# elfi-dev/elfi

Hardware: AMD Instinct MI355X
Metric: ABC distances/sec (higher is better)
Workload: dtype f64; 1 GPU; configs[1]: synthetic Gaussian summaries, 1000000 samples x 32 summaries per GPU per step, elfi.Distance('euclidean'), inputs resident in HBM; samples_per_gpu=1000000, summaries=32, layout=row-major (n,m) f64, batches_in_rotation=3, exchange=none (N = 1), exchange_every=8, world_size_seen=1

## Files before the change

### elfi_amd/csrc/adaptive.hip

```cpp
#include "common.hpp"
#include "tile_stream.hpp"
#include "internal.hpp"
#include "dist_launch.hpp"

#include <algorithm>

#pragma clang fp contract(off)

namespace elfihip {

constexpr int ADA_T = 256;
constexpr int ADA_U = 8;
constexpr int ADA_RMAX = 128;
constexpr int ADA_OCC = 4;

struct AdaptArgs {
  RowArgs A;
  const double* acc;
  unsigned long long* acc_count;
  double* partial;
};

struct ColStat {
  double n, mean, M2;
};

__device__ __forceinline__ void chan_merge(ColStat& a, double nb, double mb, double qb) {
  if (nb == 0.0) return;
  if (a.n == 0.0) {
    a.n = nb;
    a.mean = mb;
    a.M2 = qb;
    return;
  }
  const double tot = a.n + nb;
  const double delta = mb - a.mean;
  const double f = nb / tot;
  a.M2 = a.M2 + qb + delta * delta * (a.n * f);
  a.mean = a.mean + delta * f;
  a.n = tot;
}

typedef const double __attribute__((address_space(4))) * cdptr;
__device__ __forceinline__ cdptr as_constant(const double* p) { return (cdptr) reinterpret_cast<uintptr_t>(p); }

template <int B, bool PRE>
__device__ __forceinline__ double row_distance(const double* row, cdptr ys, cdptr w, int m) {
  double s = 0.0;
  double wn[B], yn[PRE ? 1 : B];
#pragma unroll
  for (int i = 0; i < B; ++i) {
    wn[i] = w[i];
    if constexpr (!PRE) yn[i] = ys[i];
  }
  double xn[4];
#pragma unroll
  for (int i = 0; i < 4; ++i) xn[i] = row[i];
  int j0 = 0;
  for (; j0 + B <= m; j0 += B) {
    double wc[B], yc[PRE ? 1 : B];
#pragma unroll
    for (int i = 0; i < B; ++i) {
      wc[i] = wn[i];
      if constexpr (!PRE) yc[i] = yn[i];
    }
    const int jn = j0 + 2 * B <= m ? j0 + B : j0;
#pragma unroll
    for (int i = 0; i < B; ++i) {
      wn[i] = w[jn + i];
      if constexpr (!PRE) yn[i] = ys[jn + i];
    }
#pragma unroll
    for (int i0 = 0; i0 < B; i0 += 4) {
      double x[4];
#pragma unroll
      for (int i = 0; i < 4; ++i) x[i] = xn[i];
#pragma unroll
      for (int i = 0; i < 4; ++i) xn[i] = row[j0 + i0 + 4 + i];
#pragma unroll
      for (int i = 0; i < 4; ++i) {
        double d = x[i];
        if constexpr (!PRE) d = d - yc[i0 + i];
        const double d2 = d * d;
        s = s + wc[i0 + i] * d2;
      }
    }
  }
  for (int j = j0; j < m; ++j) {
    double d = row[j];
    if constexpr (!PRE) d = d - ys[j];
    const double d2 = d * d;
    s = s + w[j] * d2;
  }
  return sqrt(s);
}

template <int CH>
__device__ __forceinline__ void chunk_stats(const double (&x)[CH], double& mean, double& q) {
  if constexpr (CH >= 4) {
    double a[4] = {0.0, 0.0, 0.0, 0.0};
#pragma unroll
    for (int i = 0; i < CH; i += 4) {
      a[0] += x[i];
      a[1] += x[i + 1];
      a[2] += x[i + 2];
      a[3] += x[i + 3];
    }
    mean = ((a[0] + a[1]) + (a[2] + a[3])) * (1.0 / CH);
    double b[4] = {0.0, 0.0, 0.0, 0.0};
#pragma unroll
    for (int i = 0; i < CH; i += 4) {
#pragma unroll
      for (int u = 0; u < 4; ++u) {
        const double e = x[i + u] - mean;
        b[u] += e * e;
      }
    }
    q = (b[0] + b[1]) + (b[2] + b[3]);
  } else {
    double a = 0.0;
#pragma unroll
    for (int i = 0; i < CH; ++i) a += x[i];
    mean = a * (1.0 / CH);
    q = 0.0;
#pragma unroll
    for (int i = 0; i < CH; ++i) {
      const double e = x[i] - mean;
      q += e * e;
    }
  }
}

template <int NU>
__global__ __launch_bounds__(ADA_T, ADA_OCC) void adaptive_pass_kernel(AdaptArgs P) {
  extern __shared__ __align__(16) double lds[];
  constexpr int U = NU > 0 ? NU : ADA_U;
  constexpr bool POW2 = NU > 0;
  const RowArgs& A = P.A;
  const int T = ADA_T, tid = threadIdx.x, m = A.m, K = A.K, R = A.R, mp = A.mp;
  double* tile = lds;
  const int tile_doubles = R * mp > 6 * T ? R * mp : 6 * T;
  double* accs = tile + tile_doubles + 8;
  int* flag = reinterpret_cast<int*>(accs + K);
  const cdptr ys = as_constant(A.y), ws = as_constant(A.aux);
  if (P.acc)
    for (int j = tid; j < K; j += T) accs[j] = P.acc[j];
  const int64_t ntiles = (A.n + R - 1) / R;
  const double inf = __longlong_as_double(0x7ff0000000000000ll);
  const double thr = A.F.thr ? *A.F.thr : inf;
  const int wave = __builtin_amdgcn_readfirstlane(tid >> 6);
  const int RB = R > 64 ? 2 : 1;
  const int CG = 4 / RB;
  const int rb = wave % RB, cg = wave / RB;
  const int rl = rb * 64 + (tid & 63);
  const bool owner = cg == (K - 1) % CG;
  unsigned long long nacc = 0;
  const int h = m >> 1;
  const int q0 = POW2 ? tid / h : 0, jj0 = POW2 ? tid - q0 * h : 0, QS = POW2 ? T / h : 1;
  const int64_t soff = (int64_t)q0 * A.ldx + 2 * jj0, sstep = (int64_t)QS * A.ldx;
  const int doff = q0 * mp + 2 * jj0, dstep = QS * mp;
  double2 yp = make_double2(0.0, 0.0);
  if constexpr (POW2) yp = make_double2(A.y[2 * jj0], A.y[2 * jj0 + 1]);
  const int G = T / m;
  const int g = tid / m, c = tid - g * m;
  const bool stats = P.partial != nullptr;
  ColStat st0 = {0.0, 0.0, 0.0}, st1 = {0.0, 0.0, 0.0};
  double2 v[U];
  auto fetch = [&](int64_t row0, int rows) {
    if constexpr (POW2) {
      const double* __restrict__ src = A.X + row0 * A.ldx + soff;
      if (rows == R) {
        if (A.nt) {
          typedef double v2d_nt __attribute__((ext_vector_type(2)));
#pragma unroll
          for (int u = 0; u < U; ++u) {
            const v2d_nt tv = __builtin_nontemporal_load(reinterpret_cast<const v2d_nt*>(src + u * sstep));
            v[u] = make_double2(tv.x, tv.y);
          }
        } else {
#pragma unroll
          for (int u = 0; u < U; ++u) v[u] = *reinterpret_cast<const double2*>(src + u * sstep);
        }
      } else {
#pragma unroll
        for (int u = 0; u < U; ++u) {
          v[u] = make_double2(0.0, 0.0);
          if (q0 + u * QS < rows) v[u] = *reinterpret_cast<const double2*>(src + u * sstep);
        }
      }
    } else {
      tile_fetch<U>(A, row0, rows, v);
    }
  };
  auto commit = [&](int rows) {
    if constexpr (POW2) {
      if (rows == R) {
#pragma unroll
        for (int u = 0; u < U; ++u) {
          double* dst = tile + doff + u * dstep;
          dst[0] = v[u].x - yp.x;
          dst[1] = v[u].y - yp.y;
        }
        if (stats) {
          double a[U], b[U], ma, qa, mb, qb;
#pragma unroll
          for (int u = 0; u < U; ++u) {
            a[u] = v[u].x;
            b[u] = v[u].y;
          }
          chunk_stats<U>(a, ma, qa);
          chunk_stats<U>(b, mb, qb);
          chan_merge(st0, (double)U, ma, qa);
          chan_merge(st1, (double)U, mb, qb);
        }
      } else {
        int cnt = 0;
        double sa = 0.0, sb = 0.0;
#pragma unroll
        for (int u = 0; u < U; ++u)
          if (q0 + u * QS < rows) {
            double* dst = tile + doff + u * dstep;
            dst[0] = v[u].x - yp.x;
            dst[1] = v[u].y - yp.y;
            sa += v[u].x;
            sb += v[u].y;
            ++cnt;
          }
        if (stats && cnt > 0) {
          const double ma = sa / (double)cnt, mb = sb / (double)cnt;
          double qa = 0.0, qb = 0.0;
#pragma unroll
          for (int u = 0; u < U; ++u)
            if (q0 + u * QS < rows) {
              const double ea = v[u].x - ma, eb = v[u].y - mb;
              qa += ea * ea;
              qb += eb * eb;
            }
          chan_merge(st0, (double)cnt, ma, qa);
          chan_merge(st1, (double)cnt, mb, qb);
        }
      }
    } else {
      tile_commit<U>(A, tile, rows, v);
    }
  };
  int64_t t = blockIdx.x;
  if (t < ntiles) fetch(t * R, (int)((A.n - t * R) < R ? (A.n - t * R) : R));
  for (; t < ntiles; t += gridDim.x) {
    const int64_t row0 = t * R;
    const int rows = (int)((A.n - row0) < R ? (A.n - row0) : R);
    __syncthreads();
    commit(rows);
    const int64_t tn = t + gridDim.x;
    if (tn < ntiles) fetch(tn * R, (int)((A.n - tn * R) < R ? (A.n - tn * R) : R));
    __syncthreads();
    double dlast = 0.0;
    bool ok = rl < rows;
    if (rl < rows) {
      const double* row = tile + (size_t)rl * mp;
      for (int k = cg; k < K; k += CG) {
        double r;
        if constexpr (POW2)
          r = row_distance<16, true>(row, ys, ws + (size_t)k * m, m);
        else
          r = row_distance<8, false>(row, ys, ws + (size_t)k * m, m);
        if (A.out) A.out[(row0 + rl) * K + k] = r;
        if (P.acc) ok = ok && r <= accs[k];
        dlast = r;
      }
    }
    if (P.acc && K > 1) {
      if (!owner) flag[cg * ADA_RMAX + rl] = ok ? 1 : 0;
      __syncthreads();
      if (owner) {
        const int ng = K < CG ? K : CG;
        for (int q = 0; q < ng; ++q)
          if (q != cg) ok = ok && flag[q * ADA_RMAX + rl] != 0;
      }
    }
    if (owner) {
      if (P.acc) nacc += (unsigned long long)__popcll(__ballot(ok));
      if (A.F.thr) reject_offer(A.F, ok && dlast < thr, dlast, A.F.row_base + row0 + rl);
    }
    if constexpr (!POW2) {
      if (stats && g < G && g < rows) {
        const double* col = tile + c;
        double sum = 0.0;
        int cnt = 0;
#pragma unroll 8
        for (int r = g; r < rows; r += G) {
          sum += col[(size_t)r * mp];
          ++cnt;
        }
        const double mt = sum / (double)cnt;
        double q = 0.0;
#pragma unroll 8
        for (int r = g; r < rows; r += G) {
          const double e = col[(size_t)r * mp] - mt;
          q += e * e;
        }
        chan_merge(st0, (double)cnt, mt, q);
      }
    }
  }
  if (stats) {
    __syncthreads();
    double* red = tile;
    const int nslot = POW2 ? QS : G;
    if constexpr (POW2) {
      double* e0 = red + 3 * ((size_t)q0 * m + 2 * jj0);
      e0[0] = st0.n, e0[1] = st0.mean, e0[2] = st0.M2;
      e0[3] = st1.n, e0[4] = st1.mean, e0[5] = st1.M2;
    } else if (g < G) {
      double* e0 = red + 3 * ((size_t)g * m + c);
      e0[0] = st0.n, e0[1] = st0.mean, e0[2] = st0.M2;
    }
    __syncthreads();
    if (tid < m) {
      ColStat a = {0.0, 0.0, 0.0};
      for (int sl = 0; sl < nslot; ++sl) {
        const double* e = red + 3 * ((size_t)sl * m + tid);
        chan_merge(a, e[0], e[1], e[2]);
      }
      double* o = P.partial + (size_t)blockIdx.x * (1 + 2 * m);
      if (tid == 0) o[0] = a.n;
      o[1 + tid] = a.mean;
      o[1 + m + tid] = a.M2;
    }
  }
  if (P.acc && (tid & 63) == 0 && nacc) atomicAdd(P.acc_count, nacc);
}

constexpr int ADA_NARROW_KMAX = 8;
constexpr int ADA_NARROW_U = 8;

template <int M, int U>
__global__ __launch_bounds__(256) void adaptive_narrow_kernel(AdaptArgs P) {
  __shared__ double rn[256], rm[256 * M], rq[256 * M];
  __shared__ __align__(16) double stage_all[4 * 64 * ADA_NARROW_KMAX];
  const RowArgs& A = P.A;
  const int tid = threadIdx.x, K = A.K;
  double* stage = stage_all + (tid >> 6) * 64 * ADA_NARROW_KMAX;
  const bool staged = A.out && (reinterpret_cast<uintptr_t>(A.out) & 15u) == 0;
  double yv[M], wv[ADA_NARROW_KMAX][M], accs[ADA_NARROW_KMAX];
#pragma unroll
  for (int j = 0; j < M; ++j) yv[j] = A.y[j];
#pragma unroll
  for (int k = 0; k < ADA_NARROW_KMAX; ++k) {
    accs[k] = (P.acc && k < K) ? P.acc[k] : 0.0;
#pragma unroll
    for (int j = 0; j < M; ++j) wv[k][j] = k < K ? A.aux[k * M + j] : 0.0;
  }
  const double inf = __longlong_as_double(0x7ff0000000000000ll);
  const double thr = A.F.thr ? *A.F.thr : inf;
  const bool stats = P.partial != nullptr;
  ColStat st[M];
#pragma unroll
  for (int j = 0; j < M; ++j) st[j] = {0.0, 0.0, 0.0};
  unsigned long long nacc = 0;
  typedef double v2d_nt __attribute__((ext_vector_type(2)));
  const int64_t per = 256 * U;
  for (int64_t base = (int64_t)blockIdx.x * per; base < A.n; base += (int64_t)gridDim.x * per) {
    double x[U][M];
#pragma unroll
    for (int u = 0; u < U; ++u) {
      const int64_t r = base + u * 256 + tid;
      const v2d_nt* src = reinterpret_cast<const v2d_nt*>(A.X + (r < A.n ? r : A.n - 1) * A.ldx);
#pragma unroll
      for (int h = 0; h < M / 2; ++h) {
        const v2d_nt t = __builtin_nontemporal_load(src + h);
        x[u][2 * h] = t.x;
        x[u][2 * h + 1] = t.y;
      }
    }
    if (stats) {
      if (base + per <= A.n) {
#pragma unroll
        for (int j = 0; j < M; ++j) {
          double col[U], mean, q;
#pragma unroll
          for (int u = 0; u < U; ++u) col[u] = x[u][j];
          chunk_stats<U>(col, mean, q);
          chan_merge(st[j], (double)U, mean, q);
        }
      } else {
        int cnt = 0;
#pragma unroll
        for (int u = 0; u < U; ++u) cnt += (base + u * 256 + tid < A.n) ? 1 : 0;
        if (cnt > 0) {
#pragma unroll
          for (int j = 0; j < M; ++j) {
            double sum = 0.0;
#pragma unroll
            for (int u = 0; u < U; ++u)
              if (base + u * 256 + tid < A.n) sum += x[u][j];
            const double mean = sum / (double)cnt;
            double q = 0.0;
#pragma unroll
            for (int u = 0; u < U; ++u)
              if (base + u * 256 + tid < A.n) {
                const double e = x[u][j] - mean;
                q += e * e;
              }
            chan_merge(st[j], (double)cnt, mean, q);
          }
        }
      }
    }
#pragma unroll
    for (int u = 0; u < U; ++u) {
      const int64_t r = base + u * 256 + tid;
      const bool live = r < A.n;
      double d2[M];
#pragma unroll
      for (int j = 0; j < M; ++j) {
        const double d = x[u][j] - yv[j];
        d2[j] = d * d;
      }
      double dlast = 0.0, dk[ADA_NARROW_KMAX];
      bool ok = live;
#pragma unroll
      for (int k = 0; k < ADA_NARROW_KMAX; ++k) {
        dk[k] = 0.0;
        if (k < K) {
          double sk = 0.0;
#pragma unroll
          for (int j = 0; j < M; ++j) sk = sk + wv[k][j] * d2[j];
          dlast = sqrt(sk);
          dk[k] = dlast;
          if (A.out && !staged && live) A.out[r * K + k] = dlast;
          if (P.acc) ok = ok && dlast <= accs[k];
        }
      }
      if (staged) {
        const int64_t r0 = base + u * 256 + (tid & ~63);
        const int64_t left = A.n - r0;
        if (left > 0) wave_store_rows<ADA_NARROW_KMAX>(stage, A.out + r0 * K, dk, K, tid & 63, left < 64 ? (int)left : 64);
      }
      if (P.acc) nacc += (unsigned long long)__popcll(__ballot(ok));
      if (A.F.thr) reject_offer(A.F, ok && dlast < thr, dlast, A.F.row_base + r);
    }
  }
  if (stats) {
    rn[tid] = st[0].n;
#pragma unroll
    for (int j = 0; j < M; ++j) {
      rm[j * 256 + tid] = st[j].mean;
      rq[j * 256 + tid] = st[j].M2;
    }
    __syncthreads();
    for (int s = 128; s > 0; s >>= 1) {
      double nb = 0.0;
      if (tid < s) nb = rn[tid + s];
      if (tid < s) {
#pragma unroll
        for (int j = 0; j < M; ++j) {
          ColStat a = {rn[tid], rm[j * 256 + tid], rq[j * 256 + tid]};
          chan_merge(a, nb, rm[j * 256 + tid + s], rq[j * 256 + tid + s]);
          rm[j * 256 + tid] = a.mean;
          rq[j * 256 + tid] = a.M2;
          if (j == M - 1) st[0].n = a.n;
        }
      }
      __syncthreads();
      if (tid < s) rn[tid] = st[0].n;
      __syncthreads();
    }
    if (tid < M) {
      double* o = P.partial + (size_t)blockIdx.x * (1 + 2 * M);
      if (tid == 0) o[0] = rn[0];
      o[1 + tid] = rm[tid * 256];
      o[1 + M + tid] = rq[tid * 256];
    }
  }
  if (P.acc && (tid & 63) == 0 && nacc) atomicAdd(P.acc_count, nacc);
}

__global__ __launch_bounds__(256) void adaptive_finish_kernel(const double* partial, int nparts, int m, double* bst,
                                                              double* state, unsigned* done) {
  __shared__ double rn[256], rm[256], rq[256];
  const int c = blockIdx.x, j = threadIdx.x, ns = 1 + 2 * m;
  ColStat a = {0.0, 0.0, 0.0};
  for (int p = j; p < nparts; p += 256) {
    const double* e = partial + (size_t)p * ns;
    chan_merge(a, e[0], e[1 + c], e[1 + m + c]);
  }
  rn[j] = a.n;
  rm[j] = a.mean;
  rq[j] = a.M2;
  __syncthreads();
  for (int s = 128; s > 0; s >>= 1) {
    if (j < s) {
      chan_merge(a, rn[j + s], rm[j + s], rq[j + s]);
      rn[j] = a.n;
      rm[j] = a.mean;
      rq[j] = a.M2;
    }
    __syncthreads();
  }
  if (j == 0) {
    if (c == 0) bst[0] = a.n;
    bst[1 + c] = a.mean;
    bst[1 + m + c] = a.M2;
    if (state) {
      const double n_old = state[0];
      ColStat f = {n_old, state[1 + c], state[1 + m + c]};
      if (n_old == 0.0) f.mean = 0.0, f.M2 = 0.0;
      chan_merge(f, a.n, a.mean, a.M2);
      state[1 + c] = f.mean;
      state[1 + m + c] = f.M2;
      const unsigned old = __hip_atomic_fetch_add(done, 1u, __ATOMIC_RELAXED, __HIP_MEMORY_SCOPE_AGENT);
      if (old + 1u == (unsigned)m) {
        state[0] = f.n;
        __hip_atomic_store(done, 0u, __ATOMIC_RELAXED, __HIP_MEMORY_SCOPE_AGENT);
      }
    }
  }
}

static size_t ada_lds_bytes(int m, int K, int R) {
  const int mp = m | 1;
  const size_t tile = std::max<size_t>((size_t)R * mp, 6 * (size_t)ADA_T);
  return (tile + 8 + (size_t)K + 2 * ADA_RMAX) * sizeof(double);
}

static int ada_rows_per_tile(int m) {
  int R = 2 * ADA_T * ADA_U / m;
  return R > ADA_RMAX ? ADA_RMAX : R;
}

static bool adaptive_narrow(const double* dX, int m, int64_t ldx, int K) {
  return (m == 2 || m == 4) && K >= 1 && K <= ADA_NARROW_KMAX && !(ldx & 1) && aligned16(dX);
}

bool adaptive_pass_supported(const double* dX, int m, int64_t ldx, int K) {
  if (adaptive_narrow(dX, m, ldx, K)) return true;
  if (m < 4 || m > ADA_T / 2 || (m & 1) || (ldx & 1) || !aligned16(dX)) return false;
  return ada_lds_bytes(m, K, ada_rows_per_tile(m)) <= 64 * 1024;
}

int adaptive_max_parts(const elfihip_ctx* ctx) { return ctx->cu_count * 8; }

int adaptive_pass_impl(elfihip_ctx* ctx, const double* dX, int64_t n, int m, int64_t ldx, const double* dy,
                       const double* dW, int K, double* dout, const RejectFilter* F, const double* dacc,
                       unsigned long long* dacc_count, double* partial, int* nparts) {
  if (nparts) *nparts = 0;
  if (n <= 0) return ELFIHIP_OK;
  AdaptArgs P;
  RowArgs& A = P.A;
  A = make_row_args(ctx, dX, n, m, ldx, dy, dW, 2.0, dout);
  A.K = K;
  A.R = ada_rows_per_tile(m);
  if (F) A.F = *F;
  P.acc = dacc;
  P.acc_count = dacc_count;
  P.partial = partial;
  if (adaptive_narrow(dX, m, ldx, K)) {
    constexpr int U = ADA_NARROW_U;
    int64_t gn = (n + 256 * U - 1) / (256 * U);
    if (gn > (int64_t)ctx->cu_count * 4) gn = (int64_t)ctx->cu_count * 4;
    if (m == 2)
      hipLaunchKernelGGL((adaptive_narrow_kernel<2, U>), dim3((unsigned)gn), dim3(256), 0, ctx->stream, P);
    else
      hipLaunchKernelGGL((adaptive_narrow_kernel<4, U>), dim3((unsigned)gn), dim3(256), 0, ctx->stream, P);
    if (nparts && partial) *nparts = (int)gn;
    return launch_status(ctx, "adaptive_narrow_kernel");
  }
  const size_t lds = ada_lds_bytes(m, K, A.R);
  const int64_t ntiles = (n + A.R - 1) / A.R;
  int per_cu = (int)((160 * 1024) / lds);
  if (per_cu > 8) per_cu = 8;
  if (per_cu < 1) per_cu = 1;
  int64_t g = (int64_t)ctx->cu_count * per_cu;
  if (g > ntiles) g = ntiles;
  if (g < 1) g = 1;
  const int h = m / 2;
  const int nu = (ADA_T % h == 0 && A.R % (ADA_T / h) == 0) ? A.R / (ADA_T / h) : 0;
#define ELFIHIP_ADA_LAUNCH(NU) \
  hipLaunchKernelGGL((adaptive_pass_kernel<NU>), dim3((unsigned)g), dim3(ADA_T), lds, ctx->stream, P)
  switch (nu) {
    case 8: ELFIHIP_ADA_LAUNCH(8); break;
    case 4: ELFIHIP_ADA_LAUNCH(4); break;
    case 2: ELFIHIP_ADA_LAUNCH(2); break;
    case 1: ELFIHIP_ADA_LAUNCH(1); break;
    default: ELFIHIP_ADA_LAUNCH(0); break;
  }
#undef ELFIHIP_ADA_LAUNCH
  if (nparts && partial) *nparts = (int)g;
  return launch_status(ctx, "adaptive_pass_kernel");
}

int adaptive_stats_finish(elfihip_ctx* ctx, const double* partial, int nparts, int m, double* bst, double* dstate) {
  if (nparts <= 0) return ELFIHIP_OK;
  if (dstate && !ctx->fold_cnt) {
    ELFIHIP_CHECK_HIP(ctx, hipMalloc(reinterpret_cast<void**>(&ctx->fold_cnt), 64));
    ELFIHIP_CHECK_HIP(ctx, hipMemsetAsync(ctx->fold_cnt, 0, 64, ctx->stream));
  }
  hipLaunchKernelGGL(adaptive_finish_kernel, dim3((unsigned)m), dim3(256), 0, ctx->stream, partial, nparts, m, bst, dstate,
                     ctx->fold_cnt);
  return launch_status(ctx, "adaptive statistics kernel");
}

}

using namespace elfihip;

extern "C" {

int elfihip_adaptive_push_dev(elfihip_ctx* ctx, elfihip_reject* state, const double* dX, int64_t n, int m, int64_t ldx,
                              const double* dy, const double* dW, int K, double* dout, double* dwelford,
                              int64_t row_base) {
  if (!ctx) return fail(nullptr, ELFIHIP_ERR_ARG, "ctx is NULL");
  ELFIHIP_REQUIRE(ctx, n >= 0 && m >= 1 && ldx >= m, "bad shape n=%lld m=%d ldx=%lld", (long long)n, m, (long long)ldx);
  ELFIHIP_REQUIRE(ctx, K >= 1 && K <= 64, "K=%d outside [1,64]", K);
  ELFIHIP_REQUIRE(ctx, n == 0 || (dX && dy && dW), "NULL data pointer");
  ELFIHIP_REQUIRE(ctx, !state || reject_ctx(state) == ctx, "the sampler state belongs to another context");
  if (n == 0) return ELFIHIP_OK;
  DeviceGuard g(ctx->device);
  return adaptive_push_impl(ctx, state, dX, n, m, ldx, dy, dW, K, dout, dwelford, row_base);
}

static int adaptive_push_host(elfihip_ctx* ctx, elfihip_reject* state, const double* X, int64_t n, int m, int64_t ldx,
                              const double* y, const double* W, int K, double* out, int64_t* count, double* mean,
                              double* M2, int64_t row_base) {
  ELFIHIP_REQUIRE(ctx, K >= 1 && K <= 64, "K=%d outside [1,64]", K);
  ELFIHIP_REQUIRE(ctx, y && W, "NULL data pointer");
  ELFIHIP_REQUIRE(ctx, (!count && !mean && !M2) || (count && mean && M2), "count / mean / M2 come together");
  ELFIHIP_REQUIRE(ctx, !state || reject_ctx(state) == ctx, "the sampler state belongs to another context");
  if (n == 0) return out ? keep_distances(ctx, nullptr, 0, K) : ELFIHIP_OK;
  DeviceGuard g(ctx->device);
  hipStream_t st = ctx->stream;
  const size_t ns = 1 + 2 * (size_t)m;
  std::vector<double> hst(ns, 0.0);
  if (count) {
    hst[0] = (double)*count;
    memcpy(&hst[1], mean, (size_t)m * sizeof(double));
    memcpy(&hst[1 + m], M2, (size_t)m * sizeof(double));
  }
  ELFIHIP_CHECK_HIP(ctx, ctx->par.reserve(((size_t)m + (size_t)K * m + ns) * sizeof(double)));
  double* dy = ctx->par.as<double>();
  double* dW = dy + m;
  double* dstate = dW + (size_t)K * m;
  ELFIHIP_CHECK_HIP(ctx, hipMemcpyAsync(dy, y, (size_t)m * sizeof(double), hipMemcpyHostToDevice, st));
  ELFIHIP_CHECK_HIP(ctx, hipMemcpyAsync(dW, W, (size_t)K * m * sizeof(double), hipMemcpyHostToDevice, st));
  if (count) ELFIHIP_CHECK_HIP(ctx, hipMemcpyAsync(dstate, hst.data(), ns * sizeof(double), hipMemcpyHostToDevice, st));
  double* dX;
  int64_t ldd;
  if (X) {
    ldd = (m + 1) & ~1;
    ELFIHIP_CHECK_HIP(ctx, ctx->in.reserve((size_t)n * ldd * sizeof(double)));
    dX = ctx->in.as<double>();
    ELFIHIP_CHECK_HIP(ctx, hipMemcpy2DAsync(dX, (size_t)ldd * sizeof(double), X, (size_t)ldx * sizeof(double),
                                            (size_t)m * sizeof(double), (size_t)n, hipMemcpyHostToDevice, st));
  } else {
    dX = ctx->rows.as<double>();
    ldd = m;
  }
  double* dout = nullptr;
  if (out) {
    ELFIHIP_CHECK_HIP(ctx, ctx->out.reserve((size_t)n * K * sizeof(double)));
    dout = ctx->out.as<double>();
  }
  ELFIHIP_TRY(adaptive_push_impl(ctx, state, dX, n, m, ldd, dy, dW, K, dout, count ? dstate : nullptr, row_base));
  if (out) {
    ELFIHIP_TRY(keep_distances(ctx, dout, n, K));
    ELFIHIP_CHECK_HIP(ctx, hipMemcpyAsync(out, dout, (size_t)n * K * sizeof(double), hipMemcpyDeviceToHost, st));
  }
  if (count) ELFIHIP_CHECK_HIP(ctx, hipMemcpyAsync(hst.data(), dstate, ns * sizeof(double), hipMemcpyDeviceToHost, st));
  ELFIHIP_CHECK_HIP(ctx, hipStreamSynchronize(st));
  if (count) {
    *count = (int64_t)hst[0];
    memcpy(mean, &hst[1], (size_t)m * sizeof(double));
    memcpy(M2, &hst[1 + m], (size_t)m * sizeof(double));
  }
  return ELFIHIP_OK;
}

int elfihip_adaptive_push(elfihip_ctx* ctx, elfihip_reject* state, const double* X, int64_t n, int m, int64_t ldx,
                          const double* y, const double* W, int K, double* out, int64_t* count, double* mean,
                          double* M2, int64_t row_base) {
  if (!ctx) return fail(nullptr, ELFIHIP_ERR_ARG, "ctx is NULL");
  ELFIHIP_REQUIRE(ctx, n >= 0 && m >= 1 && ldx >= m, "bad shape n=%lld m=%d ldx=%lld", (long long)n, m, (long long)ldx);
  ELFIHIP_REQUIRE(ctx, n == 0 || X, "NULL data pointer");
  return adaptive_push_host(ctx, state, X, n, m, ldx, y, W, K, out, count, mean, M2, row_base);
}

int elfihip_adaptive_push_kept(elfihip_ctx* ctx, elfihip_reject* state, uint64_t rows_epoch, const double* y,
                               const double* W, int K, double* out, int64_t* count, double* mean, double* M2,
                               int64_t row_base) {
  if (!ctx) return fail(nullptr, ELFIHIP_ERR_ARG, "ctx is NULL");
  if (rows_epoch != ctx->rows_epoch || (ctx->rows_n > 0 && !ctx->rows.p))
    return fail(ctx, ELFIHIP_ERR_STATE, "the kept rows are those of a later call (epoch %llu, asked for %llu)",
                (unsigned long long)ctx->rows_epoch, (unsigned long long)rows_epoch);
  return adaptive_push_host(ctx, state, nullptr, ctx->rows_n, ctx->rows_m, ctx->rows_m, y, W, K, out, count, mean, M2,
                            row_base);
}

}
```

Measured before the change: 23.31 billion distances/s.

## Stage distance outputs in LDS for coalesced double-buffered stores in adaptive pass

Per-row distances are written into a double-buffered LDS staging area, and a designated wave group flushes the previous tile to global memory with coalesced 16-byte vector stores. Output stores become nontemporal when the total output is large. The full-tile path is specialised at compile time, so the tail tile is handled outside the main loop. Paired Chan merges share the division. The aim is to cut uncoalesced strided output writes and per-iteration bounds checks, at the cost of more LDS, extra code paths and more complexity.

Measured after the change: 22.96 billion distances/s. 0.985x the previous value.

```diff
diff --git a/elfi_amd/csrc/adaptive.hip b/elfi_amd/csrc/adaptive.hip
--- a/elfi_amd/csrc/adaptive.hip
+++ b/elfi_amd/csrc/adaptive.hip
@@ -4,6 +4,7 @@
 #include "dist_launch.hpp"
 
 #include <algorithm>
+#include <type_traits>
 
 #pragma clang fp contract(off)
 
@@ -12,7 +13,9 @@
 constexpr int ADA_T = 256;
 constexpr int ADA_U = 8;
 constexpr int ADA_RMAX = 128;
+constexpr int64_t ADA_STREAM_BYTES = 128ll << 20;
 constexpr int ADA_OCC = 4;
+constexpr int ADA_STAGE_KMAX = 4;
 
 struct AdaptArgs {
   RowArgs A;
@@ -20,6 +23,13 @@
   unsigned long long* acc_count;
   double* partial;
 };
+
+__host__ __device__ inline int ada_tile_doubles(int mp, int R) { return R * mp > 6 * ADA_T ? R * mp : 6 * ADA_T; }
+__host__ __device__ inline int ada_stage_at(int mp, int K, int R) { return (ada_tile_doubles(mp, R) + 8 + K + 2 * ADA_RMAX + 1) & ~1; }
+__host__ __device__ inline int ada_stage_doubles(int K, int R) { return (R > 64 ? 2 : 1) * 64 * K; }
+__host__ __device__ inline bool ada_stage_fits(int mp, int K, int R) {
+  return K <= ADA_STAGE_KMAX && (ada_stage_at(mp, K, R) + 2 * ada_stage_doubles(K, R)) * (int)sizeof(double) <= 40 * 1024;
+}
 
 struct ColStat {
   double n, mean, M2;
@@ -41,6 +51,24 @@
   a.n = tot;
 }
 
+__device__ __forceinline__ void chan_merge_pair(ColStat& a, ColStat& b, double nb, double ma, double qa, double mb, double qb) {
+  if (nb == 0.0) return;
+  if (a.n == 0.0) {
+    a.n = nb, a.mean = ma, a.M2 = qa;
+    b.n = nb, b.mean = mb, b.M2 = qb;
+    return;
+  }
+  const double tot = a.n + nb;
+  const double f = nb / tot, nf = a.n * f;
+  const double da = ma - a.mean, db = mb - b.mean;
+  a.M2 = a.M2 + qa + da * da * nf;
+  b.M2 = b.M2 + qb + db * db * nf;
+  a.mean = a.mean + da * f;
+  b.mean = b.mean + db * f;
+  a.n = tot;
+  b.n = tot;
+}
+
 typedef const double __attribute__((address_space(4))) * cdptr;
 __device__ __forceinline__ cdptr as_constant(const double* p) { return (cdptr) reinterpret_cast<uintptr_t>(p); }
 
@@ -131,7 +159,7 @@
   }
 }
 
-template <int NU>
+template <int NU, bool STREAM>
 __global__ __launch_bounds__(ADA_T, ADA_OCC) void adaptive_pass_kernel(AdaptArgs P) {
   extern __shared__ __align__(16) double lds[];
   constexpr int U = NU > 0 ? NU : ADA_U;
@@ -139,9 +167,11 @@
   const RowArgs& A = P.A;
   const int T = ADA_T, tid = threadIdx.x, m = A.m, K = A.K, R = A.R, mp = A.mp;
   double* tile = lds;
-  const int tile_doubles = R * mp > 6 * T ? R * mp : 6 * T;
+  const int tile_doubles = ada_tile_doubles(mp, R);
   double* accs = tile + tile_doubles + 8;
   int* flag = reinterpret_cast<int*>(accs + K);
+  double* stage = lds + ada_stage_at(mp, K, R);
+  const int stage_doubles = ada_stage_doubles(K, R);
   const cdptr ys = as_constant(A.y), ws = as_constant(A.aux);
   if (P.acc)
     for (int j = tid; j < K; j += T) accs[j] = P.acc[j];
@@ -154,6 +184,14 @@
   const int rb = wave % RB, cg = wave / RB;
   const int rl = rb * 64 + (tid & 63);
   const bool owner = cg == (K - 1) % CG;
+  auto put = [&](auto val, auto* dst) {
+    if constexpr (STREAM)
+      __builtin_nontemporal_store(val, dst);
+    else
+      *dst = val;
+  };
+  const bool staged = POW2 && A.out != nullptr && ada_stage_fits(mp, K, R);
+  const bool storer = staged && cg == K % CG;
   unsigned long long nacc = 0;
   const int h = m >> 1;
   const int q0 = POW2 ? tid / h : 0, jj0 = POW2 ? tid - q0 * h : 0, QS = POW2 ? T / h : 1;
@@ -166,10 +204,10 @@
   const bool stats = P.partial != nullptr;
   ColStat st0 = {0.0, 0.0, 0.0}, st1 = {0.0, 0.0, 0.0};
   double2 v[U];
-  auto fetch = [&](int64_t row0, int rows) {
+  auto fetch = [&](auto full, int64_t row0, int rows) {
     if constexpr (POW2) {
       const double* __restrict__ src = A.X + row0 * A.ldx + soff;
-      if (rows == R) {
+      if constexpr (decltype(full)::value) {
         if (A.nt) {
           typedef double v2d_nt __attribute__((ext_vector_type(2)));
 #pragma unroll
@@ -192,9 +230,9 @@
       tile_fetch<U>(A, row0, rows, v);
     }
   };
-  auto commit = [&](int rows) {
+  auto commit = [&](auto full, int rows) {
     if constexpr (POW2) {
-      if (rows == R) {
+      if constexpr (decltype(full)::value) {
 #pragma unroll
         for (int u = 0; u < U; ++u) {
           double* dst = tile + doff + u * dstep;
@@ -210,8 +248,7 @@
           }
           chunk_stats<U>(a, ma, qa);
           chunk_stats<U>(b, mb, qb);
-          chan_merge(st0, (double)U, ma, qa);
-          chan_merge(st1, (double)U, mb, qb);
+          chan_merge_pair(st0, st1, (double)U, ma, qa, mb, qb);
         }
       } else {
         int cnt = 0;
@@ -236,24 +273,69 @@
               qa += ea * ea;
               qb += eb * eb;
             }
-          chan_merge(st0, (double)cnt, ma, qa);
-          chan_merge(st1, (double)cnt, mb, qb);
+          chan_merge_pair(st0, st1, (double)cnt, ma, qa, mb, qb);
         }
       }
     } else {
       tile_commit<U>(A, tile, rows, v);
     }
   };
-  int64_t t = blockIdx.x;
-  if (t < ntiles) fetch(t * R, (int)((A.n - t * R) < R ? (A.n - t * R) : R));
-  for (; t < ntiles; t += gridDim.x) {
-    const int64_t row0 = t * R;
-    const int rows = (int)((A.n - row0) < R ? (A.n - row0) : R);
-    __syncthreads();
-    commit(rows);
-    const int64_t tn = t + gridDim.x;
-    if (tn < ntiles) fetch(tn * R, (int)((A.n - tn * R) < R ? (A.n - tn * R) : R));
-    __syncthreads();
+  typedef double v2d_st __attribute__((ext_vector_type(2)));
+  v2d_st sb[ADA_STAGE_KMAX / 2];
+  auto flush_geom = [&](int64_t frow0, int frows, int& total, double*& dst) {
+    const int nv = frows - rb * 64 < 64 ? frows - rb * 64 : 64;
+    total = nv > 0 ? nv * K : 0;
+    dst = A.out + (frow0 + rb * 64) * K;
+  };
+  auto flush_take = [&](int64_t frow0, int frows, int buf) {
+    int total;
+    double* dst;
+    flush_geom(frow0, frows, total, dst);
+    const int lane = tid & 63;
+    const double* src = stage + buf * stage_doubles + rb * 64 * K;
+    if ((reinterpret_cast<uintptr_t>(dst) & 15u) == 0) {
+      const int last = (total >> 1) - 1;
+      if (last >= 0) {
+#pragma unroll
+        for (int i = 0; i < ADA_STAGE_KMAX / 2; ++i) {
+          const int p = lane + 64 * i;
+          sb[i] = *reinterpret_cast<const v2d_st*>(src + 2 * (p < last ? p : last));
+        }
+      }
+    }
+  };
+  auto flush_put = [&](int64_t frow0, int frows, int buf) {
+    int total;
+    double* dst;
+    flush_geom(frow0, frows, total, dst);
+    const int lane = tid & 63;
+    const double* src = stage + buf * stage_doubles + rb * 64 * K;
+    if ((reinterpret_cast<uintptr_t>(dst) & 15u) == 0) {
+      const int npieces = total >> 1;
+#pragma unroll
+      for (int i = 0; i < ADA_STAGE_KMAX / 2; ++i)
+        if (lane + 64 * i < npieces) put(sb[i], reinterpret_cast<v2d_st*>(dst + 2 * (lane + 64 * i)));
+      if ((total & 1) && lane == 0) put(src[total - 1], dst + total - 1);
+    } else if (total > 0) {
+      double b[ADA_STAGE_KMAX];
+#pragma unroll
+      for (int i = 0; i < ADA_STAGE_KMAX; ++i) {
+        const int p = lane + 64 * i;
+        b[i] = src[p < total ? p : total - 1];
+      }
+#pragma unroll
+      for (int i = 0; i < ADA_STAGE_KMAX; ++i)
+        if (lane + 64 * i < total) put(b[i], dst + lane + 64 * i);
+    }
+  };
+  int64_t prow0 = 0;
+  int prows = 0;
+  int par = 0;
+  auto sweep = [&](int64_t row0, int rows) {
+    if (storer && prows) {
+      flush_take(prow0, prows, par ^ 1);
+      flush_put(prow0, prows, par ^ 1);
+    }
     double dlast = 0.0;
     bool ok = rl < rows;
     if (rl < rows) {
@@ -264,7 +346,10 @@
           r = row_distance<16, true>(row, ys, ws + (size_t)k * m, m);
         else
           r = row_distance<8, false>(row, ys, ws + (size_t)k * m, m);
-        if (A.out) A.out[(row0 + rl) * K + k] = r;
+        if (staged)
+          stage[par * stage_doubles + rl * K + k] = r;
+        else if (A.out)
+          put(r, &A.out[(row0 + rl) * K + k]);
         if (P.acc) ok = ok && r <= accs[k];
         dlast = r;
       }
@@ -302,9 +387,41 @@
         chan_merge(st0, (double)cnt, mt, q);
       }
     }
+    prow0 = row0;
+    prows = rows;
+    par ^= 1;
+  };
+  const std::true_type full;
+  const int64_t nloop = POW2 ? A.n / R : ntiles;
+  int64_t t = blockIdx.x;
+  if (t < nloop) fetch(full, t * R, POW2 ? R : (int)((A.n - t * R) < R ? (A.n - t * R) : R));
+  for (; t < nloop; t += gridDim.x) {
+    const int64_t row0 = t * R;
+    const int rows = POW2 ? R : (int)((A.n - row0) < R ? (A.n - row0) : R);
+    __syncthreads();
+    commit(full, rows);
+    const int64_t tn = t + gridDim.x;
+    if (tn < nloop) fetch(full, tn * R, POW2 ? R : (int)((A.n - tn * R) < R ? (A.n - tn * R) : R));
+    __syncthreads();
+    sweep(row0, rows);
+  }
+  if constexpr (POW2) {
+    if (t == nloop && t < ntiles) {
+      const int64_t row0 = t * R;
+      const int rows = (int)(A.n - row0);
+      fetch(std::false_type(), row0, rows);
+      __syncthreads();
+      commit(std::false_type(), rows);
+      __syncthreads();
+      sweep(row0, rows);
+    }
+  }
+  __syncthreads();
+  if (storer && prows) {
+    flush_take(prow0, prows, par ^ 1);
+    flush_put(prow0, prows, par ^ 1);
   }
   if (stats) {
-    __syncthreads();
     double* red = tile;
     const int nslot = POW2 ? QS : G;
     if constexpr (POW2) {
@@ -518,10 +635,16 @@
   }
 }
 
-static size_t ada_lds_bytes(int m, int K, int R) {
+static int ada_loads_per_tile(int m, int R) {
+  const int h = m / 2;
+  return (ADA_T % h == 0 && R % (ADA_T / h) == 0) ? R / (ADA_T / h) : 0;
+}
+
+static size_t ada_lds_bytes(int m, int K, int R, bool stage) {
   const int mp = m | 1;
-  const size_t tile = std::max<size_t>((size_t)R * mp, 6 * (size_t)ADA_T);
-  return (tile + 8 + (size_t)K + 2 * ADA_RMAX) * sizeof(double);
+  const size_t d = stage ? (size_t)ada_stage_at(mp, K, R) + 2 * (size_t)ada_stage_doubles(K, R)
+                         : (size_t)ada_tile_doubles(mp, R) + 8 + (size_t)K + 2 * ADA_RMAX;
+  return d * sizeof(double);
 }
 
 static int ada_rows_per_tile(int m) {
@@ -536,7 +659,7 @@
 bool adaptive_pass_supported(const double* dX, int m, int64_t ldx, int K) {
   if (adaptive_narrow(dX, m, ldx, K)) return true;
   if (m < 4 || m > ADA_T / 2 || (m & 1) || (ldx & 1) || !aligned16(dX)) return false;
-  return ada_lds_bytes(m, K, ada_rows_per_tile(m)) <= 64 * 1024;
+  return ada_lds_bytes(m, K, ada_rows_per_tile(m), false) <= 64 * 1024;
 }
 
 int adaptive_max_parts(const elfihip_ctx* ctx) { return ctx->cu_count * 8; }
@@ -566,18 +689,24 @@
     if (nparts && partial) *nparts = (int)gn;
     return launch_status(ctx, "adaptive_narrow_kernel");
   }
-  const size_t lds = ada_lds_bytes(m, K, A.R);
+  const bool staged = dout != nullptr && ada_loads_per_tile(m, A.R) > 0 && ada_stage_fits(m | 1, K, A.R);
+  const size_t lds = ada_lds_bytes(m, K, A.R, staged);
   const int64_t ntiles = (n + A.R - 1) / A.R;
-  int per_cu = (int)((160 * 1024) / lds);
+  int per_cu = (int)((160 * 1024) / ada_lds_bytes(m, K, A.R, false));
   if (per_cu > 8) per_cu = 8;
   if (per_cu < 1) per_cu = 1;
   int64_t g = (int64_t)ctx->cu_count * per_cu;
   if (g > ntiles) g = ntiles;
   if (g < 1) g = 1;
-  const int h = m / 2;
-  const int nu = (ADA_T % h == 0 && A.R % (ADA_T / h) == 0) ? A.R / (ADA_T / h) : 0;
-#define ELFIHIP_ADA_LAUNCH(NU) \
-  hipLaunchKernelGGL((adaptive_pass_kernel<NU>), dim3((unsigned)g), dim3(ADA_T), lds, ctx->stream, P)
+  const int nu = ada_loads_per_tile(m, A.R);
+  const bool stream = dout != nullptr && n * K * (int64_t)sizeof(double) >= ADA_STREAM_BYTES;
+#define ELFIHIP_ADA_LAUNCH(NU)                                                                                       \
+  do {                                                                                                               \
+    if (stream)                                                                                                      \
+      hipLaunchKernelGGL((adaptive_pass_kernel<NU, true>), dim3((unsigned)g), dim3(ADA_T), lds, ctx->stream, P);     \
+    else                                                                                                             \
+      hipLaunchKernelGGL((adaptive_pass_kernel<NU, false>), dim3((unsigned)g), dim3(ADA_T), lds, ctx->stream, P);    \
+  } while (0)
   switch (nu) {
     case 8: ELFIHIP_ADA_LAUNCH(8); break;
     case 4: ELFIHIP_ADA_LAUNCH(4); break;
```
